# zhenpeiyang/RelativePose

Hardware: AMD Instinct MI355X
Metric: scan-pairs/sec end-to-end (completion+feat+spectral-match), 160x640 RGB-D (higher is better)
Workload: dtype f32 (fp32 products emulated on the bf16 matrix pipe: every operand cut into 3 bf16 pieces = its full 24 significand bits, the 6 partial products >= 2^-16 |ab| issued as v_mfma_f32_32x32x16_bf16, the 3 smallest dropped: a product error <= 2^-23 |ab| worst case, rms 2^-27.4 -- an fp32 multiply's own r

## Files before the change

include/relpose.h:

```cpp
#ifndef RELPOSE_H
#define RELPOSE_H

#include <stddef.h>
#include <stdint.h>

#ifdef __cplusplus
extern "C" {
#endif

#define RELPOSE_EINVAL (-1)
#define RELPOSE_ENOMEM (-2)
#define RELPOSE_EROUNDS (-3)

enum {
    RELPOSE_OK = 0,
    RELPOSE_FEW_KEYPOINTS = 1,
    RELPOSE_DIST_FILTER = 2,
    RELPOSE_ANGLE_FILTER = 3,
    RELPOSE_ZERO_WEIGHT = 4,
    RELPOSE_EDGE_OVERFLOW = 5,
    RELPOSE_NOT_CONVERGED = 6
};

enum { RELPOSE_SUNCG = 0, RELPOSE_MATTERPORT = 1, RELPOSE_SCANNET = 2 };
// ... 718 lines not shown
} RelposeSCNetConfig;
RelposeSCNet* relpose_scnet_create_ex(const RelposeSCNetConfig* cfg);

int relpose_scnet_set_param(RelposeSCNet* net, const char* key, const float* data_host, size_t numel);
int relpose_scnet_finalize(RelposeSCNet* net);
int64_t relpose_scnet_num_params(const RelposeSCNet* net);

enum { RELPOSE_PREC_F32 = 0, RELPOSE_PREC_BF16X3 = 1, RELPOSE_PREC_F16X3 = 2, RELPOSE_PREC_F16 = 3, RELPOSE_PREC_BF16X9 = 4, RELPOSE_PREC_BF16X6 = 5 };
int relpose_scnet_set_precision(RelposeSCNet* net, int32_t mode);

size_t relpose_scnet_workspace_bytes(const RelposeSCNet* net, int32_t n_images, int32_t H, int32_t W);

int relpose_scnet_forward(RelposeSCNet* net, const float* x, float* out, int32_t n_images, int32_t H, int32_t W,
                          void* workspace, size_t workspace_bytes, void* stream);

enum { RELPOSE_FWD_ZERO_WARP = 1, RELPOSE_FWD_POSE_OUTPUTS = 2, RELPOSE_FWD_NEW_WORKSPACE = 4 };
typedef struct RelposeForwardArgs {
    uint32_t struct_size;
    int32_t flags;
    const float* x;
    float* out;
    int32_t n_images, H, W, reserved0;
    void* workspace;
    size_t workspace_bytes;
    void* stream;
    void* tail_stream;
    uint64_t self_tag;
    uint64_t workspace_generation;
    void* reserved1;
} RelposeForwardArgs;
int relpose_scnet_forward_ex(RelposeSCNet* net, const RelposeForwardArgs* args);

int relpose_scnet_plan_macs(RelposeSCNet* net, int32_t n_images, int32_t flags, int32_t self_cached, double* macs_host);

int relpose_scnet_layer_kernel(RelposeSCNet* net, const char* layer, int32_t n_images);

int relpose_scnet_zero_tiles(RelposeSCNet* net, void* workspace, void* stream, int64_t* counts_host);

int relpose_scnet_conv1_zero(RelposeSCNet* net, void* workspace, void* stream, int64_t* counts_host, uint32_t* occ_host);

int relpose_scnet_conv4_rows(RelposeSCNet* net, void* workspace, void* stream, int64_t* counts_host);

int64_t relpose_scnet_read_tap(RelposeSCNet* net, const char* layer, float* out, void* workspace, void* stream);

int relpose_scnet_profile(RelposeSCNet* net, const float* x, float* out, int32_t n_images, int32_t H, int32_t W,
                          void* workspace, size_t workspace_bytes, int32_t iters,
// ... 7 lines not shown
```

relativepose_amd/_lib.py:

```python
import ctypes as C
import os

HERE = os.path.dirname(os.path.abspath(__file__))
LIB_PATH = os.environ.get("RELPOSE_LIB_PATH") or os.path.join(HERE, "librelpose_hip.so")

c_void_p, c_int, c_int64, c_size_t, c_double, c_char_p = C.c_void_p, C.c_int32, C.c_int64, C.c_size_t, C.c_double, C.c_char_p


class Params(C.Structure):
    _fields_ = [("distThre", c_double), ("distSepThre", c_double), ("angleThre", c_double),
                ("sigmaAngle1", c_double), ("sigmaAngle2", c_double), ("sigmaDist", c_double),
                ("sigmaFeat", c_double), ("mu", c_double), ("topK", c_int), ("method", c_int)]


class Keypoints(C.Structure):
    _fields_ = [("B", c_int), ("ns_max", c_int), ("nt_max", c_int),
                ("ns", c_void_p), ("nt", c_void_p),
                ("pc_s", c_void_p), ("normal_s", c_void_p), ("feat_s", c_void_p), ("weight_s", c_void_p),
                ("pc_t", c_void_p), ("normal_t", c_void_p), ("feat_t", c_void_p), ("weight_t", c_void_p)]


class MatchDebug(C.Structure):
    _fields_ = [("wij", c_void_p), ("corres_j", c_void_p), ("corres_w", c_void_p),
                ("counts", c_void_p), ("trace", c_void_p), ("eig_iters", c_void_p)]


class ForwardArgs(C.Structure):
    _fields_ = [("struct_size", C.c_uint32), ("flags", c_int), ("x", c_void_p), ("out", c_void_p),
                ("n_images", c_int), ("H", c_int), ("W", c_int), ("reserved0", c_int),
                ("workspace", c_void_p), ("workspace_bytes", c_size_t), ("stream", c_void_p), ("tail_stream", c_void_p),
                ("self_tag", C.c_uint64), ("workspace_generation", C.c_uint64), ("reserved1", c_void_p)]


class SCNetConfig(C.Structure):
    _fields_ = [("struct_size", C.c_uint32), ("snumclass", c_int), ("use_tanh", c_int), ("batchnorm", c_int), ("skip_layer", c_int),
                ("output_mask", c_int)]


class MatchArgs(C.Structure):
    _fields_ = [("struct_size", C.c_uint32), ("fit_cluster", c_int), ("params_host", C.POINTER(Params)), ("kp_host", C.POINTER(Keypoints)),
                ("workspace", c_void_p), ("workspace_bytes", c_size_t), ("max_edges", c_int64), ("pose", c_void_p), ("status", c_void_p),
                ("debug_host", C.POINTER(MatchDebug)), ("stream", c_void_p), ("affinity_kernel", c_int), ("reserved0", c_int)]


class SiftArgs(C.Structure):
    _fields_ = [("struct_size", C.c_uint32), ("n_views", c_int), ("images", c_void_p), ("img_h", c_int), ("img_w", c_int), ("channels", c_int),
# ... 275 lines not shown
    "relpose_pose_sync_workspace": (c_size_t, [c_int, c_int, c_int]),
    "relpose_pose_sync": (c_int, [C.POINTER(PoseSyncArgs)]),
    "relpose_scnet_create": (c_void_p, [c_int, c_int]),
    "relpose_scnet_create_ex": (c_void_p, [C.POINTER(SCNetConfig)]),
    "relpose_scnet_destroy": (None, [c_void_p]),
    "relpose_scnet_set_param": (c_int, [c_void_p, c_char_p, c_void_p, c_size_t]),
    "relpose_scnet_finalize": (c_int, [c_void_p]),
    "relpose_scnet_set_precision": (c_int, [c_void_p, c_int]),
    "relpose_scnet_num_params": (c_int64, [c_void_p]),
    "relpose_scnet_workspace_bytes": (c_size_t, [c_void_p, c_int, c_int, c_int]),
    "relpose_scnet_forward": (c_int, [c_void_p, c_void_p, c_void_p, c_int, c_int, c_int, c_void_p, c_size_t, c_void_p]),
    "relpose_scnet_forward_ex": (c_int, [c_void_p, C.POINTER(ForwardArgs)]),
    "relpose_scnet_plan_macs": (c_int, [c_void_p, c_int, c_int, c_int, C.POINTER(c_double)]),
    "relpose_scnet_layer_kernel": (c_int, [c_void_p, c_char_p, c_int]),
    "relpose_scnet_zero_tiles": (c_int, [c_void_p, c_void_p, c_void_p, C.POINTER(c_int64)]),
    "relpose_scnet_conv1_zero": (c_int, [c_void_p, c_void_p, c_void_p, C.POINTER(c_int64), c_void_p]),
    "relpose_scnet_conv4_rows": (c_int, [c_void_p, c_void_p, c_void_p, C.POINTER(c_int64)]),
    "relpose_scnet_read_tap": (c_int64, [c_void_p, c_char_p, c_void_p, c_void_p, c_void_p]),
    "relpose_scnet_profile": (c_int, [c_void_p, c_void_p, c_void_p, c_int, c_int, c_int, c_void_p, c_size_t, c_int,
                                      C.POINTER(c_double), C.POINTER(c_double), C.POINTER(c_int64), c_void_p]),
}

_lib = None


def lib():
    global _lib
    if _lib is None:
        if not os.path.exists(LIB_PATH):
            _build_locked()
# ... 71 lines not shown
```

relativepose_amd/csrc/geometry.hip:

```cpp
#include "common.h"
#include "rp_math.h"
#include "skybox.h"
#include <limits.h>

namespace {

struct Box { int y0, y1, x0, x1; };
__host__ __device__ inline Box observed_box(int method, int h) {
    Box b;
    if (method == RELPOSE_MASK_SECOND) { b.y0 = 0; b.y1 = h; b.x0 = h; b.x1 = 2 * h; }
    else {
        int dw = (int)(44 * (h / 160.0)), dh = (int)(33 * (h / 160.0));
        b.y0 = h / 2 - dh; b.y1 = h / 2 + dh; b.x0 = h + h / 2 - dw; b.x1 = h + h / 2 + dw;
    }
    return b;
}

__global__ void apply_mask_kernel(float* x, float* mask, int n, int c, int h, Box bx) {
    const size_t hw = (size_t)h * 4 * h;
    const size_t total = (size_t)n * hw;
    for (size_t idx = (size_t)blockIdx.x * blockDim.x + threadIdx.x; idx < total; idx += (size_t)gridDim.x * blockDim.x) {
        const size_t img = idx / hw, p = idx - img * hw;
        const int y = (int)(p / (4 * h)), xx = (int)(p - (size_t)y * 4 * h);
        const float m = (y >= bx.y0 && y < bx.y1 && xx >= bx.x0 && xx < bx.x1) ? 1.0f : 0.0f;
// ... 176 lines not shown

__global__ void sample_primitives_kernel(const float* __restrict__ f, int cf, int feat_off, const float* __restrict__ obs_norm,
                                         const float* __restrict__ obs_depth, const double* __restrict__ pts,
                                         const int* __restrict__ npts, int npts_max, double* __restrict__ pc,
                                         double* __restrict__ normal, float* __restrict__ feat, int n, int h, Box bx, int dataset,
                                         int compose) {
    const int img = blockIdx.y;
    const int k = blockIdx.x * blockDim.x + threadIdx.x;
    if (k >= npts[img]) return;
    const size_t hw = (size_t)h * 4 * h;
    const int W = 4 * h;
    const float* fi = f + (size_t)img * cf * hw;
    const float* on = obs_norm + (size_t)img * 3 * hw;
    const float* od = obs_depth + (size_t)img * hw;
    const double px = pts[((size_t)img * npts_max + k) * 2 + 0], py = pts[((size_t)img * npts_max + k) * 2 + 1];
    const int tx = (int)floor(px), ty = (int)floor(py);
    const double fx1 = px - tx, fx0 = tx + 1 - px, fy1 = py - ty, fy0 = ty + 1 - py;
    float n00[3], n01[3], n10[3], n11[3], d00, d01, d10, d11;
    composed_pixel(fi, cf, on, od, hw, h, bx, compose, ty, tx, n00, d00);
    composed_pixel(fi, cf, on, od, hw, h, bx, compose, ty, tx + 1, n01, d01);
    composed_pixel(fi, cf, on, od, hw, h, bx, compose, ty + 1, tx, n10, d10);
    composed_pixel(fi, cf, on, od, hw, h, bx, compose, ty + 1, tx + 1, n11, d11);
    const double val = (((double)d00 * fy0 * fx0 + (double)d01 * fx1 * fy0) + (double)d10 * fy1 * fx0) + (double)d11 * fx1 * fy1;
    double nn[3];
#pragma unroll
    for (int a = 0; a < 3; ++a)
        nn[a] = (((double)n00[a] * fy0 * fx0 + (double)n01[a] * fx1 * fy0) + (double)n10[a] * fy1 * fx0) + (double)n11[a] * fx1 * fy1;
    const double nl = rp_norm3(nn[0], nn[1], nn[2]);
    double* no = normal + ((size_t)img * npts_max + k) * 3;
    no[0] = nn[0] / nl; no[1] = nn[1] / nl; no[2] = nn[2] / nl;
    const int slot = (int)floor(px / h);
    const double ystp = (0.5 - py / h) * 2, xstp = ((px - slot * h) / h - 0.5) * 2;
    double ox, oy, oz;
    rp_face_rot(rp_face_index(dataset, slot), xstp * val, ystp * val, -val, ox, oy, oz);
    double* po = pc + ((size_t)img * npts_max + k) * 3;
    po[0] = ox; po[1] = oy; po[2] = oz;
    const float ptx = (float)(px / W), pty = (float)(py / h);
    const float x = ptx * (float)(W - 1), y = pty * (float)(h - 1);
    const float x0 = floorf(x), y0 = floorf(y);
    const int xi = (int)x0, yi = (int)y0;
    const float wx0 = x0 + 1.0f - x, wy0 = y0 + 1.0f - y, wx1 = x - x0, wy1 = y - y0;
    const float* ff = fi + (size_t)feat_off * hw;
    float* fo = feat + ((size_t)img * npts_max + k) * 32;
    for (int c = 0; c < 32; ++c) {
        const float* fc = ff + (size_t)c * hw;
        const float v00 = fc[(size_t)yi * W + xi], v10 = fc[(size_t)(yi + 1) * W + xi];
        const float v01 = fc[(size_t)yi * W + xi + 1], v11 = fc[(size_t)(yi + 1) * W + xi + 1];
        fo[c] = ((v00 * wx0 * wy0 + v10 * wx0 * wy1) + v01 * wx1 * wy0) + v11 * wx1 * wy1;
    }
}

__global__ void get_pixel_kernel(const double* __restrict__ depth, const double* __restrict__ normal, const double* __restrict__ pts,
                                 int k_total, int h, int dataset, double* __restrict__ pc, double* __restrict__ nn_out) {
    const int k = blockIdx.x * blockDim.x + threadIdx.x;
    if (k >= k_total) return;
// ... 321 lines not shown
```

relativepose_amd/csrc/scnet.hip:

```cpp
#include "common.h"
#include "matcher_internal.h"
#include "conv1_zero_geom.h"
#include <map>
#include <string>
#include <vector>
#include <algorithm>
#include <math.h>
#include <stdio.h>
#include <string.h>
#include <type_traits>
#include <stdlib.h>
#include <stddef.h>

namespace {

typedef float floatx16 __attribute__((ext_vector_type(16)));
typedef __bf16 bf16x8 __attribute__((ext_vector_type(8)));
typedef __bf16 bf16x4 __attribute__((ext_vector_type(4)));
typedef _Float16 f16x8 __attribute__((ext_vector_type(8)));
typedef _Float16 f16x4 __attribute__((ext_vector_type(4)));
template <int SPLIT> struct SplitT { typedef bf16x8 v8; typedef bf16x4 v4; };
template <> struct SplitT<2> { typedef f16x8 v8; typedef f16x4 v4; };
template <> struct SplitT<3> { typedef f16x8 v8; typedef f16x4 v4; };
typedef float rp_f4v __attribute__((ext_vector_type(4)));
// ... 2373 lines not shown
        if (ox < W) {
            int x0, x1; float lx0, lx1;
            lin_coef(ox, sww, RS, x0, x1, lx0, lx1);
            const float* a = srow + (x0 - g.sx) * C;
            const float* b = srow + (x1 - g.sx) * C;
            const float* cc = a + RO_MAXW * C;
            const float* dd = b + RO_MAXW * C;
            float* o = y + (size_t)g.img * C * H * W + (size_t)g.oy * W + ox;
            for (int c = 0; c < C; ++c)
                o[(size_t)c * H * W] = g.ly0 * (lx0 * a[c] + lx1 * b[c]) + g.ly1 * (lx0 * cc[c] + lx1 * dd[c]);
        }
        __builtin_amdgcn_wave_barrier();
    }
}

struct Phase {
    int ntaps; signed char offy[16], offx[16];
    int py, px, Hp, Wp;
    size_t w_off;
    size_t ws_off = 0;
    size_t wh_off = 0;
    float wh_scale = 1.f;
    size_t w3_off = 0;
    int K;
};

struct Layer {
    std::string name;
    int kind;
    int cin, cout, k, stride, pad;
// ... 9 lines not shown
struct RelposeSCNet {
    int S, use_tanh, cf;
    int bn = 1, skip = 1, omask = 31;
    bool variant() const { return !(bn && skip && omask == 31); }
    std::map<std::string, std::vector<float>> params;
    std::map<std::string, std::vector<int64_t>> shapes;
    bool finalized = false;
    int prec = 0;
    int64_t nparams = 0;
    float* d_w = nullptr;
    float* d_gb = nullptr;
    float2* d_ident = nullptr;
    size_t w1_off = 0;
    size_t wh_off = 0, bh_off = 0;
    std::map<std::pair<void*, int64_t>, void*> plans;
    struct SelfState { uint64_t tag = 0, gen = 0; int n = 0, H = 0, W = 0; int snap_heads = 0; bool c4_rows = false; };
    std::map<void*, SelfState> self_state;
    std::map<std::string, Layer> layers;
    std::map<std::string, Buf> bufs;
    size_t per_image_floats = 0, ss_float2_per_group = 0;
    size_t gb_floats = 0;
    int last_n = 0;
    const int* last_zt_counts = nullptr;
    const int* last_c4_hdr = nullptr;
    int last_c4_nimg[6] = {0, 0, 0, 0, 0, 0};
    int64_t last_zt_units[2] = {0, 0};
    bool w1_finite = false;
    struct A1zState { uint64_t gen = 0; int n = 0, H = 0, W = 0; };
    std::map<void*, A1zState> a1z_state;
    int64_t last_c1_units = 0;
    bool last_c1_codes = false, last_occ = false;
    bool profiling = false;
    std::vector<hipEvent_t> ev;
    std::vector<int> ev_kind;
};

namespace {
// ... 903 lines not shown
                          size_t workspace_bytes, void* stream) {
    const RelposeForwardArgs a = rp_fwd_args(x, out, n, H, W, workspace, workspace_bytes, stream, stream, 0, 0);
    return relpose_scnet_forward_ex(net, &a);
}

int relpose_scnet_forward_ex(RelposeSCNet* net, const RelposeForwardArgs* args) {
    if (!net || !args || args->struct_size < offsetof(RelposeForwardArgs, self_tag)) return RELPOSE_EINVAL;
    const float* x = args->x; float* out = args->out;
    const int32_t n = args->n_images, H = args->H, W = args->W, flags = args->flags;
    void* workspace = args->workspace; const size_t workspace_bytes = args->workspace_bytes;
    const bool variant = net->variant();
    void* stream = args->stream; void* tail_stream = (args->tail_stream && !variant) ? args->tail_stream : args->stream;
    const uint64_t self_tag = (!variant && args->struct_size >= offsetof(RelposeForwardArgs, self_tag) + sizeof(uint64_t)) ? args->self_tag : 0;
    const uint64_t ws_gen = args->struct_size >= offsetof(RelposeForwardArgs, workspace_generation) + sizeof(uint64_t) ? args->workspace_generation : 0;
    if (!net->finalized || !x || !out || !workspace || n <= 0 || (n & 1) || H <= 0 || W <= 0 || n >= (1 << 24)) return RELPOSE_EINVAL;
    if (flags & ~(RELPOSE_FWD_ZERO_WARP | RELPOSE_FWD_POSE_OUTPUTS | RELPOSE_FWD_NEW_WORKSPACE)) return RELPOSE_EINVAL;
    if (args->struct_size >= offsetof(RelposeForwardArgs, reserved1) + sizeof(void*) && args->reserved1) return RELPOSE_EINVAL;
    const int G = n / 2;
    const bool zero_warp = (flags & RELPOSE_FWD_ZERO_WARP) && n > 2 && !variant;
    const bool pose_only = (flags & RELPOSE_FWD_POSE_OUTPUTS) != 0 && !variant;
    Plan* plan = nullptr;
    RelposeSCNet::SelfState commit;
    const bool zt_on = g_rp_tune[RELPOSE_TUNE_ZERO_TILES] != 1;
    const bool c4_on = zt_on && g_rp_tune[RELPOSE_TUNE_CONV4_ROWS] != 1;
    commit.c4_rows = c4_on;
    commit.tag = self_tag; commit.n = n; commit.H = H; commit.W = W; commit.gen = ws_gen;
    if (flags & RELPOSE_FWD_NEW_WORKSPACE) net->self_state.erase(workspace);
    RelposeSCNet::SelfState prev = net->self_state[workspace];
    net->self_state[workspace] = RelposeSCNet::SelfState();
    bool self_cached = self_tag != 0 && prev.tag == self_tag && prev.n == n && prev.H == H && prev.W == W && (prev.snap_heads & 6) == 6 && !zero_warp &&
                       prev.gen == ws_gen && prev.c4_rows == c4_on;
    int snap_mode = 0, snap_heads = 7;
    const int ds_key = ((g_rp_tune[RELPOSE_TUNE_DECONV_STRIP] == 1 ? 1 : 0) << 28) | ((zt_on ? 0 : 1) << 29) | ((c4_on ? 0 : 1) << 30);
    auto key_of = [&]() {
        return (int64_t)((int)n | (zero_warp ? 1 << 24 : 0) | (pose_only ? 1 << 25 : 0) | (self_cached ? 1 << 26 : 0) | (snap_mode == 1 ? 1 << 27 : 0) | ds_key) |
// ... 22 lines not shown
        B.zt = zt_on ? (int*)(ws + o.zt) + zt_occ_ints(n) : nullptr;
        B.c4r = c4_on ? (int*)(ws + o.c4r) : nullptr;
        build_plan(net, n, B);
        if (B.rc) {
            delete p;
            if (self_cached) { self_cached = false; continue; }
            return B.rc;
        }
        RP_HIP(hipMalloc((void**)&p->d_descs, MAX_DESCS * sizeof(ConvDesc)));
        RP_HIP(hipMemcpy(p->d_descs, p->descs.data(), p->descs.size() * sizeof(ConvDesc), hipMemcpyHostToDevice));
        net->plans[std::make_pair(workspace, key_of())] = p;
        plan = p;
    }
    if (!plan) return RELPOSE_EINVAL;
    commit.snap_heads = plan->self_cached ? prev.snap_heads : (self_tag != 0 ? (pose_only ? 6 : 7) : 0);
    net->last_n = n;
    const bool two = tail_stream != stream;
    hipStream_t s = (two && plan->head_count > 0) ? (hipStream_t)tail_stream : (hipStream_t)stream;
    const WsOffsets o = ws_offsets(net, n);
    char* ws = (char*)workspace;
    float* act = (float*)(ws + o.act);
    float2* ssp = (float2*)(ws + o.ss);
    double* partial = (double*)(ws + o.partial);
    auto mark = [&](int kind) {
        if (!net->profiling) return;
        hipEvent_t e; (void)hipEventCreate(&e); (void)hipEventRecord(e, s);
        net->ev.push_back(e); net->ev_kind.push_back(kind);
    };
    if (net->omask != 31) {
        for (const char* bn_ : {"D3", "D2", "OUT"}) {
            const Buf& B = net->bufs[bn_];
// ... 170 lines not shown
            mark(2);
            hipLaunchKernelGGL(bn_finalize_fused_kernel, dim3((B.C + 31) / 32, G), dim3(1024), 0, s, plan->d_descs + op.first, op.count, op.skip_blk,
                               B.C, 2 * B.H * B.H, net->d_gb + B.gb_off, net->d_gb + B.gb_off + B.C, ssp + B.ss_off * G);
            mark(-2);
        } else if (op.type == OP_SS_FILL) {
            const Buf& B = net->bufs[op.buf];
            mark(2);
            hipLaunchKernelGGL(ss_fill_kernel, dim3((B.C * G + 255) / 256), dim3(256), 0, s, B.C, G, net->d_gb + B.gb_off, net->d_gb + B.gb_off + B.C,
                               ssp + B.ss_off * G);
            mark(-2);
        } else if (op.type == OP_BCAST) {
            const Buf& B = net->bufs[op.buf];
            mark(2);
            hipLaunchKernelGGL(bcast_warped_kernel, dim3(2048), dim3(256), 0, s, act + B.off * n, n, B.H * B.H, B.C, B.C / 6, ssp + B.ss_off * G, G);
            mark(-2);
        } else if (op.type == OP_HEADS) {
            HeadsDesc hd;
            hd.d2 = act + net->bufs["D2"].off * n; hd.a1 = act + net->bufs["A1"].off * n;
            hd.ss_d2 = ssp + net->bufs["D2"].ss_off * G; hd.ss_a1 = ssp + net->bufs["A1"].ss_off * G;
            hd.w = net->d_w + net->wh_off; hd.bias = net->d_w + net->bh_off; hd.out = act + net->bufs["OUT"].off * n;
            hd.n = n; hd.S = net->S; hd.cf = net->cf; hd.use_tanh = net->use_tanh;
            hd.snap_mode = plan->snap_mode; hd.snap = (float*)(ws + o.snap) + plan->heads_snap_off; hd.snap_heads = plan->snap_heads;
            mark(1);
            const dim3 hg((unsigned)((size_t)n * RS * RS / 256));
#define RP_HEADS_LAUNCH(S_, POSE_)                                                                                         \
            { if (lanepix) hipLaunchKernelGGL((heads_lanepix_kernel<S_, POSE_>), hg, dim3(256), 0, s, hd);               \
              else hipLaunchKernelGGL((heads_kernel<S_, POSE_>), hg, dim3(256), 0, s, hd); }
            const bool lanepix = g_rp_tune[RELPOSE_TUNE_HEADS_KERNEL] == 1;
            if (plan->pose_only) {
                if (net->S == 15) RP_HEADS_LAUNCH(15, true) else RP_HEADS_LAUNCH(21, true)
            } else if (net->S == 15) RP_HEADS_LAUNCH(15, false) else RP_HEADS_LAUNCH(21, false)
#undef RP_HEADS_LAUNCH
            mark(-1);
        } else if (op.type == OP_REDUCE) {
            mark(4);
            if (op.cfg == 1) {
                const ConvDesc& d0 = plan->descs[op.first];
// ... 22 lines not shown
            int nch = (2048 + G - 1) / G;
            if (nch > (rows + 63) / 64) nch = (rows + 63) / 64;
            if (nch > 64) nch = 64;
            if (nch < 1) nch = 1;
            const int chunk_rows = (rows + nch - 1) / nch;
            nch = (rows + chunk_rows - 1) / chunk_rows;
            const int q4 = B.C / 4, nrl = 256 / q4;
            mark(2);
            hipLaunchKernelGGL(bn_partial_kernel, dim3(nch, G), dim3(256), (size_t)nrl * q4 * 8 * sizeof(double), s, act + B.off * n, rows,
                               B.C, chunk_rows, partial);
            hipLaunchKernelGGL(bn_finalize_kernel, dim3((B.C + 255) / 256, G), dim3(256), 0, s, partial, nch, B.C, rows,
                               net->d_gb + B.gb_off, net->d_gb + B.gb_off + B.C, ssp + B.ss_off * G);
            mark(-2);
        }
    }
    mark(3);
    hipLaunchKernelGGL(resize_out_kernel, dim3(4096), dim3(256), net->cf <= RO_MAXC ? (size_t)4 * 2 * RO_MAXW * net->cf * sizeof(float) : 0, s,
                       act + net->bufs["OUT"].off * n, out, n, net->cf, H, W);
    mark(-3);
    RP_CHECK_LAUNCH();
    {
        net->self_state[workspace] = commit;
        if (net->last_c1_codes) {
            RelposeSCNet::A1zState z; z.gen = ws_gen; z.n = n; z.H = H; z.W = W;
            net->a1z_state[workspace] = z;
        }
    }
    return 0;
}

int relpose_scnet_plan_macs(RelposeSCNet* net, int32_t n, int32_t flags, int32_t self_cached, double* macs_out) {
    if (!net || !net->finalized || !macs_out || n <= 0 || (n & 1)) return RELPOSE_EINVAL;
    if (net->variant()) { flags = 0; self_cached = 0; }
    const bool zero_warp = (flags & RELPOSE_FWD_ZERO_WARP) && n > 2 && !self_cached;
    const bool pose_only = (flags & RELPOSE_FWD_POSE_OUTPUTS) != 0;
    Plan dry;
    Builder B; B.net = net; B.n = n; B.G = n / 2; B.act = nullptr; B.ss = nullptr; B.splitk = nullptr; B.statp = nullptr; B.plan = &dry;
    B.zero_warp = zero_warp; B.pose_only = pose_only; B.self_cached = self_cached != 0;
    B.snapbuf = (float*)(uintptr_t)4096;
    B.snap_mode = self_cached ? 2 : 1; dry.snap_mode = B.snap_mode;
    const int snap_heads = self_cached == 2 ? 6 : 7;
    B.snap_heads = snap_heads; dry.snap_heads = snap_heads;
    build_plan(net, n, B);
    if (B.rc) return B.rc;
    double macs = 0;
    for (const Op& op : dry.ops) {
        if (op.type == OP_CONV || op.type == OP_CONV_S2 || op.type == OP_CONV_STRIP || op.type == OP_DECONV_TILE) {
            for (int i = op.first; i < op.first + op.count; ++i) {
                const ConvDesc& d = dry.descs[i];
                double rowsK;
                if (op.type == OP_CONV_STRIP && d.ksplit > 1 && (d.shared_slices || d.skip_slices)) {
                    rowsK = 0;
                    for (int ks = 0; ks < d.ksplit; ++ks) {
                        if ((d.skip_slices >> ks) & 1) continue;
                        const double rows = ((d.shared_slices >> ks) & 1) ? 2.0 * d.Hp * d.Wp : (double)d.M;
                        rowsK += rows * d.K / d.ksplit;
                    }
                } else if (op.type == OP_DECONV_TILE && d.nsrc == 2 && plan_snap_mode(dry, i) == 2) {
                    rowsK = (double)d.M * d.ntaps * d.src[0].C;
                } else rowsK = (double)d.M * d.K;
                macs += rowsK * d.Cout;
            }
        } else if (op.type == OP_CONV1) {
            const double blk = 224.0 * 224 * 32 * (36 + 36 + 18);
            const double self_imgs = self_cached ? 0 : n, warp_imgs = zero_warp ? 2 : n;
            macs += blk * (self_imgs + warp_imgs);
        } else if (op.type == OP_HEADS) {
            const double px = (double)n * 224 * 224;
            const int hc[5] = {3, 3, 1, net->S, 32};
            for (int m = 0; m < 5; ++m) {
                if (pose_only && (m == 0 || m == 3)) continue;
                const int cin = (m < 3 && self_cached && ((snap_heads >> m) & 1)) ? 32 : 64;
                macs += px * cin * hc[m];
            }
        }
    }
    *macs_out = macs;
    return 0;
}

int relpose_scnet_layer_kernel(RelposeSCNet* net, const char* layer, int32_t n) {
    if (!net || !net->finalized || !layer || n <= 0 || (n & 1)) return RELPOSE_EINVAL;
    Plan dry;
    Builder B; B.net = net; B.n = n; B.G = n / 2; B.act = nullptr; B.ss = nullptr; B.splitk = nullptr; B.statp = nullptr; B.plan = &dry;
    B.probe_layer = layer;
    build_plan(net, n, B);
    if (B.rc) return B.rc;
    if (B.probe_desc < 0) return RELPOSE_EINVAL;
    for (const Op& op : dry.ops)
        if ((op.type == OP_CONV || op.type == OP_CONV_S2 || op.type == OP_CONV_STRIP || op.type == OP_DECONV_TILE) && B.probe_desc >= op.first &&
            B.probe_desc < op.first + op.count)
            return (op.type == OP_CONV_STRIP && op.cfg == 1) ? (dry.descs[B.probe_desc].ksplit == 1 ? 2 : 1) : 0;
    return RELPOSE_EINVAL;
}
// ... 103 lines not shown
```

relativepose_amd/model.py:

```python
import ctypes as C

import numpy as np
import torch

from . import _lib
from .weights import HEADS, head_channels, parse_output_type, state_dict_spec

PRECISION_CODES = {"f32": 0, "bf16x3": 1, "f16x3": 2, "f16": 3, "bf16x9": 4, "bf16x6": 5}

BUFFER_SHAPES = {"X0": (224, 16), "A1": (224, 192), "A2": (112, 384), "A3": (56, 768), "A4": (28, 256), "A5": (14, 512),
                 "A6": (7, 512), "A7": (3, 512), "A8": (3, 512), "A9": (1, 1024), "D9": (3, 512), "D8": (3, 512),
                 "D7": (7, 512), "D6": (14, 512), "D5": (28, 256), "D4": (56, 128), "D3": (112, 320), "D2": (224, 224)}


_REGISTRY = {}


class SCNet(torch.nn.Module):

    def __init__(self, args):
        super().__init__()
        self.snumclass = int(args.snumclass)
        self.useTanh = int(getattr(args, "useTanh", 1))
        self.batchnorm = int(bool(getattr(args, "batchnorm", 1)))
# ... 102 lines not shown
        self._wss[key] = ent
        ws, self._ws_gen = ent
        ws.record_stream(torch.cuda.current_stream())
        for s in also_streams:
            ws.record_stream(s)
        self._ws, self._ws_n = ws, n
        return ws

    _tag_counter = 0

    @classmethod
    def new_self_tag(cls):
        cls._tag_counter += 1
        return cls._tag_counter

    FLAG_ZERO_WARP, FLAG_POSE_OUTPUTS, FLAG_NEW_WORKSPACE = 1, 2, 4

    def forward(self, x, out=None, tail_stream=None, ws_key=None, zero_warp=False, outputs="all", self_tag=0):
        flags = (self.FLAG_ZERO_WARP if zero_warp else 0) | {"all": 0, "pose": self.FLAG_POSE_OUTPUTS}[outputs]
        return self.forward_flags(x, out, flags, self_tag, tail_stream, ws_key)

    def forward_flags(self, x, out=None, flags=0, self_tag=0, tail_stream=None, ws_key=None):
        import torch
        _lib.require_gpu()
        if not self._loaded:
            raise RuntimeError("load_state_dict first")
        assert x.is_cuda and x.dtype == torch.float32 and x.dim() == 4 and x.shape[1] == 16
        x = x.contiguous()
        n, _, H, W = x.shape
        if isinstance(tail_stream, int):
            tail_stream = None if tail_stream == 0 else torch.cuda.ExternalStream(tail_stream)
        ws = self._workspace(n, H, W, x.device, ws_key, tuple(s_ for s_ in (tail_stream,) if s_ is not None))
        if tail_stream is not None:
            x.record_stream(tail_stream)
        user_out = None
        if self.is_variant:
            tail_stream, user_out = None, out
            out = torch.empty(n, self.full_channels, H, W, dtype=torch.float32, device=x.device)
        elif out is None:
            out = torch.empty(n, self.out_channels, H, W, dtype=torch.float32, device=x.device)
            if tail_stream is not None:
                out.record_stream(tail_stream)
        else:
            assert out.is_cuda and out.dtype == torch.float32 and out.is_contiguous() and tuple(out.shape) == (n, self.out_channels, H, W)
        a = _lib.ForwardArgs()
        a.struct_size = C.sizeof(_lib.ForwardArgs)
        a.flags = int(flags) & 7
        a.x, a.out = x.data_ptr(), out.data_ptr()
        a.n_images, a.H, a.W = n, H, W
        a.workspace, a.workspace_bytes = ws.data_ptr(), ws.numel()
        a.stream = torch.cuda.current_stream().cuda_stream
        a.tail_stream = a.stream if tail_stream is None else tail_stream.cuda_stream
        a.self_tag = int(self_tag)
        a.workspace_generation = self._ws_gen
        _lib.check(_lib.lib().relpose_scnet_forward_ex(self._h, C.byref(a)), "relpose_scnet_forward_ex")
        if self.is_variant:
            sel = out if self.out_channels == self.full_channels else out[:, self._sel]
            if user_out is None:
                return sel.contiguous()
            user_out.copy_(sel)
            return user_out
        return out
# ... 59 lines not shown
```

relativepose_amd/pipeline.py:

```python
import numpy as np

from . import _lib, rpmodule, util


class RelativePosePipeline:
    _chain_nets = False
    _net_stream = None
    _net_streams = None

    def __init__(self, net, dataset="suncg", mask_method="second", sigmas=None, alter_steps=3, completion=1, max_edges=0, compose=0, outputs="all",
                 self_stream_cache=True, tail_overlap=True, net_priority=None, loop_fit_cluster=1, keypoints="given", level_outputs="last"):
        self.net = net
        if keypoints not in ("given", "reference"):
            raise ValueError("keypoints must be 'given' or 'reference'")
        self.keypoints = keypoints
        self.self_stream_cache = self_stream_cache
        self.outputs = outputs
        if level_outputs not in ("last", "every"):
            raise ValueError("level_outputs must be 'last' or 'every'")
        self.level_outputs = level_outputs
        self.dataset = dataset
        self.mask_method = mask_method
        self.alter_steps = alter_steps
        self.completion = completion
        self.max_edges = max_edges
        self.compose = compose
        if sigmas is None:
            o = rpmodule.opts()
            sigmas = [[o.sigmaAngle1, o.sigmaAngle2, o.sigmaDist, o.sigmaFeat]] * alter_steps
        self.sigmas = np.asarray(sigmas, dtype=np.float64).reshape(-1, 4)
        self.feat_off = 7 + net.snumclass
        self._slot_streams = []
        self.tail_overlap = bool(tail_overlap)
        self.net_priority = net_priority
        self.loop_fit_cluster = int(loop_fit_cluster)
# ... 237 lines not shown
                        results[k] = on_result(k, pose, status)
                    else:
                        if provider is not None:
                            cur.wait_stream(st["stream"])
                            cur.wait_stream(self._net_stream)
                        results[k] = (pose, status)
        for st in states:
            if "stream" in st:
                cur.wait_stream(st["stream"])
        for ss in self._slot_streams[:depth]:
            cur.wait_stream(ss)
        cur.wait_stream(self._net_stream)
        self._chain_nets = False
        return results

    def _outputs_at(self, step, keep=None):
        if self.outputs == "all" and self.level_outputs == "last" and keep is None and step < self.alter_steps - 1 and not self.net.is_variant:
            return "pose"
        return self.outputs

    def _net_input(self, st):
        import torch
        B, h = st["B"], st["h"]
        view = util.build_view_dev(st["rgb"], st["norm"], st["depth"], self.mask_method)
        x = st.get("x")
        if x is None:
            x = st["x"] = torch.empty(2 * B, 16, h, 4 * h, dtype=torch.float32, device=view.device)
        x[:, :8].copy_(view)
        st["self_tag"] = self.net.new_self_tag() if self.self_stream_cache else 0
        f = st.get("f")
        if f is None or f.shape[1] != self.net.out_channels:
            st["f"] = torch.empty(2 * B, self.net.out_channels, h, 4 * h, dtype=torch.float32, device=view.device)
# ... 2 lines not shown
    def _run_gen(self, st):
        import torch
        B, h, N = st["B"], st["h"], st["N"]
        x = self._net_input(st)
        R_hat, status = st["eye"], None
        for step in range(self.alter_steps):
            inv = R_hat if step == 0 else util.pose_inverse_dev(R_hat)
            poses = torch.stack((inv, R_hat), 1).reshape(2 * B, 4, 4).contiguous()
            util.warp_pairs_dev(x, poses, self.dataset)
            if self._chain_nets:
                ms, ns = torch.cuda.current_stream(), self._net_stream
                ns.wait_stream(ms)
                if self.tail_overlap:
                    f = st["f"]
                    with torch.cuda.stream(ns):
                        self.net.forward(x, out=f, tail_stream=ms, ws_key=ms.cuda_stream, zero_warp=(step == 0), outputs=self._outputs_at(step),
                                         self_tag=st["self_tag"])
                else:
                    with torch.cuda.stream(ns):
                        f = self.net.forward(x, out=st["f"], zero_warp=(step == 0), outputs=self._outputs_at(step), self_tag=st["self_tag"])
                        done = torch.cuda.Event()
                        done.record()
                    ms.wait_event(done)
                yield
            else:
                f = self.net.forward(x, out=st["f"], zero_warp=(step == 0), outputs=self._outputs_at(step), self_tag=st["self_tag"])
            kpts, knpts, w_s, w_t, ns, nt = self._level_keypoints(st, f, step)
            pc, nn, ft = util.sample_primitives_dev(f, self.feat_off, st["norm"], st["depth"], kpts, knpts,
                                                    self.mask_method, self.dataset, self.compose)
            pc, nn, ft = pc.view(B, 2, N, 3), nn.view(B, 2, N, 3), ft.view(B, 2, N, 32)
            para = rpmodule.opts(*self.sigmas[min(step, len(self.sigmas) - 1)])
            res = rpmodule.match_pairs(pc[:, 0].contiguous(), nn[:, 0].contiguous(), ft[:, 0].contiguous(), w_s,
                                       pc[:, 1].contiguous(), nn[:, 1].contiguous(), ft[:, 1].contiguous(), w_t,
                                       ns, nt, para, max_edges=self.max_edges, fit_cluster=self.loop_fit_cluster if self._chain_nets else 0)
            R_hat, status = res.pose, res.status
        return R_hat, status, None

    def run(self, st, R_forced=None, keep=None, primitives=None):
        import torch
        B, h, N = st["B"], st["h"], st["N"]
        x = self._net_input(st)
        R_hat = st["eye"]
        trace = []
        status = None
        for step in range(self.alter_steps):
            if R_forced is not None:
                R_hat = R_forced[step]
            inv = R_hat if (step == 0 and R_forced is None) else util.pose_inverse_dev(R_hat)
            poses = torch.stack((inv, R_hat), 1).reshape(2 * B, 4, 4).contiguous()
            util.warp_pairs_dev(x, poses, self.dataset)
            f = self.net.forward(x, out=st["f"] if keep is None else None, zero_warp=(step == 0 and R_forced is None),
                                 outputs=self._outputs_at(step, keep), self_tag=st["self_tag"])
            kpts, knpts, w_s, w_t, ns, nt = self._level_keypoints(st, f, step)
            pc, nn, ft = util.sample_primitives_dev(f, self.feat_off, st["norm"], st["depth"], kpts, knpts,
                                                    self.mask_method, self.dataset, self.compose)
            pc, nn, ft = pc.view(B, 2, N, 3), nn.view(B, 2, N, 3), ft.view(B, 2, N, 32)
            para = rpmodule.opts(*self.sigmas[min(step, len(self.sigmas) - 1)])
            res = rpmodule.match_pairs(pc[:, 0].contiguous(), nn[:, 0].contiguous(), ft[:, 0].contiguous(), w_s,
                                       pc[:, 1].contiguous(), nn[:, 1].contiguous(), ft[:, 1].contiguous(), w_t,
                                       ns, nt, para, max_edges=self.max_edges)
            R_hat, status = res.pose, res.status
            trace.append(R_hat)
            if primitives is not None:
                primitives.update(pc=pc, nn=nn, ft=ft, step=step, w_s=w_s, w_t=w_t, ns=ns, nt=nt)
            if keep is not None:
                keep.append({"x": x.clone(), "f": f, "pc": pc, "nn": nn, "ft": ft, "pts": kpts.view(B, 2, N, 2), "w_s": w_s, "w_t": w_t, "ns": ns, "nt": nt})
        return R_hat, status, trace
# ... 1 lines not shown
```

Baseline: 1039.

## Compute output heads only at sampled keypoint pixels for intermediate levels

Adds a sampled-outputs forward mode. For non-final alternation steps it runs the normal/depth and feature heads only at the 2x2 neighbourhoods of given keypoints, through a new per-keypoint kernel, and skips the dense heads and the full-resolution resize. This removes dense head GEMMs and the resize pass over every pixel on intermediate levels. In exchange, the dense output buffer stays stale outside the sampled pixels. Heads-snapshot bookkeeping is adjusted so the next dense call does not reuse snapshots that were never produced.

```diff
diff --git a/include/relpose.h b/include/relpose.h
--- a/include/relpose.h
+++ b/include/relpose.h
@@ -756,7 +756,7 @@
 int relpose_scnet_forward(RelposeSCNet* net, const float* x, float* out, int32_t n_images, int32_t H, int32_t W,
                           void* workspace, size_t workspace_bytes, void* stream);
 
-enum { RELPOSE_FWD_ZERO_WARP = 1, RELPOSE_FWD_POSE_OUTPUTS = 2, RELPOSE_FWD_NEW_WORKSPACE = 4 };
+enum { RELPOSE_FWD_ZERO_WARP = 1, RELPOSE_FWD_POSE_OUTPUTS = 2, RELPOSE_FWD_NEW_WORKSPACE = 4, RELPOSE_FWD_SAMPLED_OUTPUTS = 32 };
 typedef struct RelposeForwardArgs {
     uint32_t struct_size;
     int32_t flags;
@@ -770,8 +770,13 @@
     uint64_t self_tag;
     uint64_t workspace_generation;
     void* reserved1;
+    const double* sample_pts;
+    const int32_t* sample_npts;
+    int32_t sample_npts_max, reserved2;
 } RelposeForwardArgs;
 int relpose_scnet_forward_ex(RelposeSCNet* net, const RelposeForwardArgs* args);
+
+int relpose_scnet_last_tail(RelposeSCNet* net);
 
 int relpose_scnet_plan_macs(RelposeSCNet* net, int32_t n_images, int32_t flags, int32_t self_cached, double* macs_host);
 
diff --git a/relativepose_amd/_lib.py b/relativepose_amd/_lib.py
--- a/relativepose_amd/_lib.py
+++ b/relativepose_amd/_lib.py
@@ -29,7 +29,8 @@
     _fields_ = [("struct_size", C.c_uint32), ("flags", c_int), ("x", c_void_p), ("out", c_void_p),
                 ("n_images", c_int), ("H", c_int), ("W", c_int), ("reserved0", c_int),
                 ("workspace", c_void_p), ("workspace_bytes", c_size_t), ("stream", c_void_p), ("tail_stream", c_void_p),
-                ("self_tag", C.c_uint64), ("workspace_generation", C.c_uint64), ("reserved1", c_void_p)]
+                ("self_tag", C.c_uint64), ("workspace_generation", C.c_uint64), ("reserved1", c_void_p),
+                ("sample_pts", c_void_p), ("sample_npts", c_void_p), ("sample_npts_max", c_int), ("reserved2", c_int)]
 
 
 class SCNetConfig(C.Structure):
@@ -335,6 +336,7 @@
     "relpose_scnet_plan_macs": (c_int, [c_void_p, c_int, c_int, c_int, C.POINTER(c_double)]),
     "relpose_scnet_layer_kernel": (c_int, [c_void_p, c_char_p, c_int]),
     "relpose_scnet_zero_tiles": (c_int, [c_void_p, c_void_p, c_void_p, C.POINTER(c_int64)]),
+    "relpose_scnet_last_tail": (c_int, [c_void_p]),
     "relpose_scnet_conv1_zero": (c_int, [c_void_p, c_void_p, c_void_p, C.POINTER(c_int64), c_void_p]),
     "relpose_scnet_conv4_rows": (c_int, [c_void_p, c_void_p, c_void_p, C.POINTER(c_int64)]),
     "relpose_scnet_read_tap": (c_int64, [c_void_p, c_char_p, c_void_p, c_void_p, c_void_p]),
diff --git a/relativepose_amd/csrc/geometry.hip b/relativepose_amd/csrc/geometry.hip
--- a/relativepose_amd/csrc/geometry.hip
+++ b/relativepose_amd/csrc/geometry.hip
@@ -1,5 +1,6 @@
 #include "common.h"
 #include "rp_math.h"
+#include "sample_pixels.h"
 #include "skybox.h"
 #include <limits.h>
 
@@ -214,7 +215,8 @@
     const float* on = obs_norm + (size_t)img * 3 * hw;
     const float* od = obs_depth + (size_t)img * hw;
     const double px = pts[((size_t)img * npts_max + k) * 2 + 0], py = pts[((size_t)img * npts_max + k) * 2 + 1];
-    const int tx = (int)floor(px), ty = (int)floor(py);
+    const RpSamplePix sp = rp_sample_pixels(px, py, h);
+    const int tx = sp.tx, ty = sp.ty;
     const double fx1 = px - tx, fx0 = tx + 1 - px, fy1 = py - ty, fy0 = ty + 1 - py;
     float n00[3], n01[3], n10[3], n11[3], d00, d01, d10, d11;
     composed_pixel(fi, cf, on, od, hw, h, bx, compose, ty, tx, n00, d00);
@@ -235,10 +237,8 @@
     rp_face_rot(rp_face_index(dataset, slot), xstp * val, ystp * val, -val, ox, oy, oz);
     double* po = pc + ((size_t)img * npts_max + k) * 3;
     po[0] = ox; po[1] = oy; po[2] = oz;
-    const float ptx = (float)(px / W), pty = (float)(py / h);
-    const float x = ptx * (float)(W - 1), y = pty * (float)(h - 1);
-    const float x0 = floorf(x), y0 = floorf(y);
-    const int xi = (int)x0, yi = (int)y0;
+    const float x = sp.x, y = sp.y, x0 = sp.x0, y0 = sp.y0;
+    const int xi = sp.xi, yi = sp.yi;
     const float wx0 = x0 + 1.0f - x, wy0 = y0 + 1.0f - y, wx1 = x - x0, wy1 = y - y0;
     const float* ff = fi + (size_t)feat_off * hw;
     float* fo = feat + ((size_t)img * npts_max + k) * 32;
diff --git a/relativepose_amd/csrc/sample_pixels.h b/relativepose_amd/csrc/sample_pixels.h
--- /dev/null
+++ b/relativepose_amd/csrc/sample_pixels.h
@@ -0,0 +1,14 @@
+#pragma once
+#include "rp_math.h"
+
+struct RpSamplePix { int tx, ty, xi, yi; float x, y, x0, y0; };
+RP_HD RpSamplePix rp_sample_pixels(double px, double py, int h) {
+    const int W = 4 * h;
+    RpSamplePix s;
+    s.tx = (int)floor(px); s.ty = (int)floor(py);
+    const float ptx = (float)(px / W), pty = (float)(py / h);
+    s.x = ptx * (float)(W - 1); s.y = pty * (float)(h - 1);
+    s.x0 = floorf(s.x); s.y0 = floorf(s.y);
+    s.xi = (int)s.x0; s.yi = (int)s.y0;
+    return s;
+}
diff --git a/relativepose_amd/csrc/scnet.hip b/relativepose_amd/csrc/scnet.hip
--- a/relativepose_amd/csrc/scnet.hip
+++ b/relativepose_amd/csrc/scnet.hip
@@ -1,6 +1,7 @@
 #include "common.h"
 #include "matcher_internal.h"
 #include "conv1_zero_geom.h"
+#include "sample_pixels.h"
 #include <map>
 #include <string>
 #include <vector>
@@ -2411,6 +2412,104 @@
     }
 }
 
+struct SampledDesc {
+    const float* d2; const float* a1; const float2* ss_d2; const float2* ss_a1;
+    const float* w; const float* bias; float* out;
+    const double* pts; const int* npts;
+    int npts_max, cf, use_tanh, H, W;
+};
+
+__global__ __launch_bounds__(256) void heads_sampled_kernel(const SampledDesc sd) {
+    __shared__ float ndl[4][16][4];
+    __shared__ float fl[4][16][32];
+    const int lane = threadIdx.x & 63, wave = threadIdx.x >> 6;
+    const int img = blockIdx.y, k = blockIdx.x * 4 + wave;
+    if (k >= sd.npts_max || k >= sd.npts[img]) return;
+    const int H = sd.H, W = sd.W, cf = sd.cf, feat_off = cf - 32;
+    const double px = sd.pts[((size_t)img * sd.npts_max + k) * 2 + 0], py = sd.pts[((size_t)img * sd.npts_max + k) * 2 + 1];
+    const RpSamplePix sp = rp_sample_pixels(px, py, H);
+    const float shh = (float)RS / H, sww = (float)RS / W;
+    const int g = img >> 1;
+    const float2* ssd = sd.ss_d2 + (size_t)g * 224;
+    const float2* ssa = sd.ss_a1 + (size_t)g * 192;
+    auto item_src = [&](int item, int by, int bx, int& oy, int& ox, size_t& spix) {
+        oy = by + (item >> 3); ox = bx + ((item >> 2) & 1);
+        if (oy < 0 || oy >= H || ox < 0 || ox >= W) return false;
+        int y0, y1, x0, x1; float ly0, ly1, lx0, lx1;
+        lin_coef(oy, shh, RS, y0, y1, ly0, ly1);
+        lin_coef(ox, sww, RS, x0, x1, lx0, lx1);
+        spix = ((size_t)img * RS + ((item & 2) ? y1 : y0)) * RS + ((item & 1) ? x1 : x0);
+        return true;
+    };
+    if (lane < 16) {
+        int oy, ox; size_t spix;
+        if (item_src(lane, sp.ty, sp.tx, oy, ox, spix)) {
+            const float* pa = sd.a1 + spix * 192;
+            const float* pd = sd.d2 + spix * 224;
+            float an[3] = {0.f, 0.f, 0.f}, ad = 0.f;
+            for (int c = 0; c < 32; ++c) {
+                const float2 sc = ssa[64 + c];
+                const float v = lrelu(pa[64 + c] * sc.x + sc.y, LRELU);
+                for (int j = 0; j < 3; ++j) an[j] = __builtin_fmaf(v, sd.w[(128 + c) * 4 + j], an[j]);
+            }
+            for (int c = 0; c < 32; ++c) {
+                const float2 sc = ssa[128 + c];
+                const float v = lrelu(pa[128 + c] * sc.x + sc.y, LRELU);
+                ad = __builtin_fmaf(v, sd.w[(160 + c) * 4], ad);
+            }
+            for (int c = 0; c < 32; ++c) {
+                const float2 sc = ssd[32 + c];
+                const float v = lrelu(pd[32 + c] * sc.x + sc.y, LRELU);
+                for (int j = 0; j < 3; ++j) an[j] = __builtin_fmaf(v, sd.w[(32 + c) * 4 + j], an[j]);
+            }
+            for (int c = 0; c < 32; ++c) {
+                const float2 sc = ssd[64 + c];
+                const float v = lrelu(pd[64 + c] * sc.x + sc.y, LRELU);
+                ad = __builtin_fmaf(v, sd.w[(64 + c) * 4], ad);
+            }
+            for (int j = 0; j < 3; ++j) ndl[wave][lane][j] = an[j] + sd.bias[3 + j];
+            ndl[wave][lane][3] = ad + sd.bias[6];
+        }
+    } else if (lane < 48) {
+        const int item = (lane - 16) & 15, o0 = ((lane - 16) >> 4) * 16;
+        int oy, ox; size_t spix;
+        if (item_src(item, sp.yi, sp.xi, oy, ox, spix)) {
+            const float* pd = sd.d2 + spix * 224 + 160;
+            const float* wf = sd.w + 2304 + o0;
+            float af[16];
+#pragma unroll
+            for (int o = 0; o < 16; ++o) af[o] = 0.f;
+            for (int c = 0; c < 64; ++c) {
+                const float2 sc = ssd[160 + c];
+                const float v = lrelu(pd[c] * sc.x + sc.y, LRELU);
+#pragma unroll
+                for (int o = 0; o < 16; ++o) af[o] = __builtin_fmaf(v, wf[c * 32 + o], af[o]);
+            }
+#pragma unroll
+            for (int o = 0; o < 16; ++o) {
+                const float v = af[o] + sd.bias[feat_off + o0 + o];
+                fl[wave][item][o0 + o] = sd.use_tanh ? tanhf(v) : v;
+            }
+        }
+    }
+    rp_wave_lds_sync();
+    const size_t hw = (size_t)H * W;
+    float* const oi = sd.out + (size_t)img * cf * hw;
+    for (int e = lane; e < 16 + 128; e += 64) {
+        const bool nd = e < 16;
+        const int p = nd ? (e >> 2) : ((e - 16) >> 5), c = nd ? (e & 3) : ((e - 16) & 31);
+        const int oy = (nd ? sp.ty : sp.yi) + (p >> 1), ox = (nd ? sp.tx : sp.xi) + (p & 1);
+        if (oy < 0 || oy >= H || ox < 0 || ox >= W) continue;
+        int y0, y1, x0, x1; float ly0, ly1, lx0, lx1;
+        lin_coef(oy, shh, RS, y0, y1, ly0, ly1);
+        lin_coef(ox, sww, RS, x0, x1, lx0, lx1);
+        const float a = nd ? ndl[wave][p * 4 + 0][c] : fl[wave][p * 4 + 0][c], b = nd ? ndl[wave][p * 4 + 1][c] : fl[wave][p * 4 + 1][c];
+        const float cc = nd ? ndl[wave][p * 4 + 2][c] : fl[wave][p * 4 + 2][c], dd = nd ? ndl[wave][p * 4 + 3][c] : fl[wave][p * 4 + 3][c];
+        const float r = __fmaf_rn(ly0, __fmaf_rn(lx0, a, __fmul_rn(lx1, b)), __fmul_rn(ly1, __fmaf_rn(lx0, cc, __fmul_rn(lx1, dd))));
+        oi[(size_t)(nd ? 3 + c : feat_off + c) * hw + (size_t)oy * W + ox] = r;
+    }
+}
+
 struct Phase {
     int ntaps; signed char offy[16], offx[16];
     int py, px, Hp, Wp;
@@ -2450,13 +2549,14 @@
     size_t w1_off = 0;
     size_t wh_off = 0, bh_off = 0;
     std::map<std::pair<void*, int64_t>, void*> plans;
-    struct SelfState { uint64_t tag = 0, gen = 0; int n = 0, H = 0, W = 0; int snap_heads = 0; bool c4_rows = false; };
+    struct SelfState { uint64_t tag = 0, gen = 0; int n = 0, H = 0, W = 0; int snap_heads = 0; int heads_snap = 0; bool c4_rows = false; };
     std::map<void*, SelfState> self_state;
     std::map<std::string, Layer> layers;
     std::map<std::string, Buf> bufs;
     size_t per_image_floats = 0, ss_float2_per_group = 0;
     size_t gb_floats = 0;
     int last_n = 0;
+    int last_tail = -1;
     const int* last_zt_counts = nullptr;
     const int* last_c4_hdr = nullptr;
     int last_c4_nimg[6] = {0, 0, 0, 0, 0, 0};
@@ -3390,11 +3490,17 @@
     const uint64_t self_tag = (!variant && args->struct_size >= offsetof(RelposeForwardArgs, self_tag) + sizeof(uint64_t)) ? args->self_tag : 0;
     const uint64_t ws_gen = args->struct_size >= offsetof(RelposeForwardArgs, workspace_generation) + sizeof(uint64_t) ? args->workspace_generation : 0;
     if (!net->finalized || !x || !out || !workspace || n <= 0 || (n & 1) || H <= 0 || W <= 0 || n >= (1 << 24)) return RELPOSE_EINVAL;
-    if (flags & ~(RELPOSE_FWD_ZERO_WARP | RELPOSE_FWD_POSE_OUTPUTS | RELPOSE_FWD_NEW_WORKSPACE)) return RELPOSE_EINVAL;
+    if (flags & ~(RELPOSE_FWD_ZERO_WARP | RELPOSE_FWD_POSE_OUTPUTS | RELPOSE_FWD_NEW_WORKSPACE | RELPOSE_FWD_SAMPLED_OUTPUTS)) return RELPOSE_EINVAL;
+    const bool sampled = (flags & RELPOSE_FWD_SAMPLED_OUTPUTS) != 0 && !variant;
+    if (flags & RELPOSE_FWD_SAMPLED_OUTPUTS) {
+        if (args->struct_size < offsetof(RelposeForwardArgs, sample_npts_max) + sizeof(int32_t)) return RELPOSE_EINVAL;
+        if (!args->sample_pts || !args->sample_npts || args->sample_npts_max <= 0 || W != 4 * H) return RELPOSE_EINVAL;
+        if (!variant && net->S != 15 && net->S != 21) return RELPOSE_EINVAL;
+    }
     if (args->struct_size >= offsetof(RelposeForwardArgs, reserved1) + sizeof(void*) && args->reserved1) return RELPOSE_EINVAL;
     const int G = n / 2;
     const bool zero_warp = (flags & RELPOSE_FWD_ZERO_WARP) && n > 2 && !variant;
-    const bool pose_only = (flags & RELPOSE_FWD_POSE_OUTPUTS) != 0 && !variant;
+    const bool pose_only = ((flags & RELPOSE_FWD_POSE_OUTPUTS) != 0 && !variant) || sampled;
     Plan* plan = nullptr;
     RelposeSCNet::SelfState commit;
     const bool zt_on = g_rp_tune[RELPOSE_TUNE_ZERO_TILES] != 1;
@@ -3447,7 +3553,9 @@
     }
     if (!plan) return RELPOSE_EINVAL;
     commit.snap_heads = plan->self_cached ? prev.snap_heads : (self_tag != 0 ? (pose_only ? 6 : 7) : 0);
+    commit.heads_snap = plan->self_cached ? prev.heads_snap : (sampled ? 0 : commit.snap_heads);
     net->last_n = n;
+    net->last_tail = sampled ? 1 : 0;
     const bool two = tail_stream != stream;
     hipStream_t s = (two && plan->head_count > 0) ? (hipStream_t)tail_stream : (hipStream_t)stream;
     const WsOffsets o = ws_offsets(net, n);
@@ -3648,6 +3756,16 @@
             mark(2);
             hipLaunchKernelGGL(bcast_warped_kernel, dim3(2048), dim3(256), 0, s, act + B.off * n, n, B.H * B.H, B.C, B.C / 6, ssp + B.ss_off * G, G);
             mark(-2);
+        } else if (op.type == OP_HEADS && sampled) {
+            SampledDesc sd;
+            sd.d2 = act + net->bufs["D2"].off * n; sd.a1 = act + net->bufs["A1"].off * n;
+            sd.ss_d2 = ssp + net->bufs["D2"].ss_off * G; sd.ss_a1 = ssp + net->bufs["A1"].ss_off * G;
+            sd.w = net->d_w + net->wh_off; sd.bias = net->d_w + net->bh_off; sd.out = out;
+            sd.pts = args->sample_pts; sd.npts = args->sample_npts; sd.npts_max = args->sample_npts_max;
+            sd.cf = net->cf; sd.use_tanh = net->use_tanh; sd.H = H; sd.W = W;
+            mark(1);
+            hipLaunchKernelGGL(heads_sampled_kernel, dim3((unsigned)((args->sample_npts_max + 3) / 4), (unsigned)n), dim3(256), 0, s, sd);
+            mark(-1);
         } else if (op.type == OP_HEADS) {
             HeadsDesc hd;
             hd.d2 = act + net->bufs["D2"].off * n; hd.a1 = act + net->bufs["A1"].off * n;
@@ -3655,6 +3773,10 @@
             hd.w = net->d_w + net->wh_off; hd.bias = net->d_w + net->bh_off; hd.out = act + net->bufs["OUT"].off * n;
             hd.n = n; hd.S = net->S; hd.cf = net->cf; hd.use_tanh = net->use_tanh;
             hd.snap_mode = plan->snap_mode; hd.snap = (float*)(ws + o.snap) + plan->heads_snap_off; hd.snap_heads = plan->snap_heads;
+            if (hd.snap_mode == 2) {
+                hd.snap_heads &= prev.heads_snap | (plan->pose_only ? 1 : 0);
+                if ((hd.snap_heads & 6) != 6) { hd.snap_mode = 0; hd.snap_heads = 7; }
+            }
             mark(1);
             const dim3 hg((unsigned)((size_t)n * RS * RS / 256));
 #define RP_HEADS_LAUNCH(S_, POSE_)                                                                                         \
@@ -3707,10 +3829,12 @@
             mark(-2);
         }
     }
-    mark(3);
-    hipLaunchKernelGGL(resize_out_kernel, dim3(4096), dim3(256), net->cf <= RO_MAXC ? (size_t)4 * 2 * RO_MAXW * net->cf * sizeof(float) : 0, s,
-                       act + net->bufs["OUT"].off * n, out, n, net->cf, H, W);
-    mark(-3);
+    if (!sampled) {
+        mark(3);
+        hipLaunchKernelGGL(resize_out_kernel, dim3(4096), dim3(256), net->cf <= RO_MAXC ? (size_t)4 * 2 * RO_MAXW * net->cf * sizeof(float) : 0, s,
+                           act + net->bufs["OUT"].off * n, out, n, net->cf, H, W);
+        mark(-3);
+    }
     RP_CHECK_LAUNCH();
     {
         net->self_state[workspace] = commit;
@@ -3726,13 +3850,15 @@
     if (!net || !net->finalized || !macs_out || n <= 0 || (n & 1)) return RELPOSE_EINVAL;
     if (net->variant()) { flags = 0; self_cached = 0; }
     const bool zero_warp = (flags & RELPOSE_FWD_ZERO_WARP) && n > 2 && !self_cached;
-    const bool pose_only = (flags & RELPOSE_FWD_POSE_OUTPUTS) != 0;
+    const bool sampled = (flags & RELPOSE_FWD_SAMPLED_OUTPUTS) != 0;
+    const bool pose_only = (flags & RELPOSE_FWD_POSE_OUTPUTS) != 0 || sampled;
     Plan dry;
     Builder B; B.net = net; B.n = n; B.G = n / 2; B.act = nullptr; B.ss = nullptr; B.splitk = nullptr; B.statp = nullptr; B.plan = &dry;
     B.zero_warp = zero_warp; B.pose_only = pose_only; B.self_cached = self_cached != 0;
     B.snapbuf = (float*)(uintptr_t)4096;
     B.snap_mode = self_cached ? 2 : 1; dry.snap_mode = B.snap_mode;
-    const int snap_heads = self_cached == 2 ? 6 : 7;
+    const int snap_heads = (self_cached == 2 || self_cached == 3) ? 6 : 7;
+    const int heads_snap = self_cached == 3 ? 0 : snap_heads;
     B.snap_heads = snap_heads; dry.snap_heads = snap_heads;
     build_plan(net, n, B);
     if (B.rc) return B.rc;
@@ -3758,12 +3884,12 @@
             const double blk = 224.0 * 224 * 32 * (36 + 36 + 18);
             const double self_imgs = self_cached ? 0 : n, warp_imgs = zero_warp ? 2 : n;
             macs += blk * (self_imgs + warp_imgs);
-        } else if (op.type == OP_HEADS) {
+        } else if (op.type == OP_HEADS && !sampled) {
             const double px = (double)n * 224 * 224;
             const int hc[5] = {3, 3, 1, net->S, 32};
             for (int m = 0; m < 5; ++m) {
                 if (pose_only && (m == 0 || m == 3)) continue;
-                const int cin = (m < 3 && self_cached && ((snap_heads >> m) & 1)) ? 32 : 64;
+                const int cin = (m < 3 && self_cached && ((heads_snap >> m) & 1)) ? 32 : 64;
                 macs += px * cin * hc[m];
             }
         }
@@ -3771,6 +3897,8 @@
     *macs_out = macs;
     return 0;
 }
+
+int relpose_scnet_last_tail(RelposeSCNet* net) { return net ? net->last_tail : RELPOSE_EINVAL; }
 
 int relpose_scnet_layer_kernel(RelposeSCNet* net, const char* layer, int32_t n) {
     if (!net || !net->finalized || !layer || n <= 0 || (n & 1)) return RELPOSE_EINVAL;
diff --git a/relativepose_amd/model.py b/relativepose_amd/model.py
--- a/relativepose_amd/model.py
+++ b/relativepose_amd/model.py
@@ -140,13 +140,19 @@
         cls._tag_counter += 1
         return cls._tag_counter
 
-    FLAG_ZERO_WARP, FLAG_POSE_OUTPUTS, FLAG_NEW_WORKSPACE = 1, 2, 4
-
-    def forward(self, x, out=None, tail_stream=None, ws_key=None, zero_warp=False, outputs="all", self_tag=0):
-        flags = (self.FLAG_ZERO_WARP if zero_warp else 0) | {"all": 0, "pose": self.FLAG_POSE_OUTPUTS}[outputs]
-        return self.forward_flags(x, out, flags, self_tag, tail_stream, ws_key)
-
-    def forward_flags(self, x, out=None, flags=0, self_tag=0, tail_stream=None, ws_key=None):
+    FLAG_ZERO_WARP, FLAG_POSE_OUTPUTS, FLAG_NEW_WORKSPACE, FLAG_SAMPLED_OUTPUTS = 1, 2, 4, 32
+
+    def forward(self, x, out=None, tail_stream=None, ws_key=None, zero_warp=False, outputs="all", self_tag=0, sample_pts=None, sample_npts=None):
+        flags = (self.FLAG_ZERO_WARP if zero_warp else 0) | {"all": 0, "pose": self.FLAG_POSE_OUTPUTS, "samples": self.FLAG_SAMPLED_OUTPUTS}[outputs]
+        if outputs == "samples" and (sample_pts is None or sample_npts is None):
+            raise ValueError("outputs='samples' needs sample_pts and sample_npts")
+        return self.forward_flags(x, out, flags, self_tag, tail_stream, ws_key, sample_pts if outputs == "samples" else None, sample_npts)
+
+    def last_tail(self):
+        r = int(_lib.lib().relpose_scnet_last_tail(self._h))
+        return {0: "dense", 1: "sampled"}.get(r)
+
+    def forward_flags(self, x, out=None, flags=0, self_tag=0, tail_stream=None, ws_key=None, sample_pts=None, sample_npts=None):
         import torch
         _lib.require_gpu()
         if not self._loaded:
@@ -171,7 +177,17 @@
             assert out.is_cuda and out.dtype == torch.float32 and out.is_contiguous() and tuple(out.shape) == (n, self.out_channels, H, W)
         a = _lib.ForwardArgs()
         a.struct_size = C.sizeof(_lib.ForwardArgs)
-        a.flags = int(flags) & 7
+        a.flags = int(flags) & (7 | self.FLAG_SAMPLED_OUTPUTS)
+        if a.flags & self.FLAG_SAMPLED_OUTPUTS:
+            if sample_pts is None or sample_npts is None:
+                raise ValueError("RELPOSE_FWD_SAMPLED_OUTPUTS needs sample_pts and sample_npts")
+            assert sample_pts.is_cuda and sample_pts.dtype == torch.float64 and sample_pts.is_contiguous() and sample_pts.dim() == 3
+            assert tuple(sample_pts.shape) == (n, sample_pts.shape[1], 2) and sample_pts.shape[1] > 0
+            assert sample_npts.is_cuda and sample_npts.dtype == torch.int32 and sample_npts.is_contiguous() and tuple(sample_npts.shape) == (n,)
+            a.sample_pts, a.sample_npts, a.sample_npts_max = sample_pts.data_ptr(), sample_npts.data_ptr(), int(sample_pts.shape[1])
+            if tail_stream is not None:
+                sample_pts.record_stream(tail_stream)
+                sample_npts.record_stream(tail_stream)
         a.x, a.out = x.data_ptr(), out.data_ptr()
         a.n_images, a.H, a.W = n, H, W
         a.workspace, a.workspace_bytes = ws.data_ptr(), ws.numel()
diff --git a/relativepose_amd/pipeline.py b/relativepose_amd/pipeline.py
--- a/relativepose_amd/pipeline.py
+++ b/relativepose_amd/pipeline.py
@@ -9,7 +9,8 @@
     _net_streams = None
 
     def __init__(self, net, dataset="suncg", mask_method="second", sigmas=None, alter_steps=3, completion=1, max_edges=0, compose=0, outputs="all",
-                 self_stream_cache=True, tail_overlap=True, net_priority=None, loop_fit_cluster=1, keypoints="given", level_outputs="last"):
+                 self_stream_cache=True, tail_overlap=True, net_priority=None, loop_fit_cluster=1, keypoints="given", level_outputs="last",
+                 sampled_levels=True):
         self.net = net
         if keypoints not in ("given", "reference"):
             raise ValueError("keypoints must be 'given' or 'reference'")
@@ -19,6 +20,7 @@
         if level_outputs not in ("last", "every"):
             raise ValueError("level_outputs must be 'last' or 'every'")
         self.level_outputs = level_outputs
+        self.sampled_levels = bool(sampled_levels)
         self.dataset = dataset
         self.mask_method = mask_method
         self.alter_steps = alter_steps
@@ -286,8 +288,10 @@
         self._chain_nets = False
         return results
 
-    def _outputs_at(self, step, keep=None):
+    def _outputs_at(self, step, keep=None, st=None):
         if self.outputs == "all" and self.level_outputs == "last" and keep is None and step < self.alter_steps - 1 and not self.net.is_variant:
+            if self.sampled_levels and self.keypoints == "given" and st is not None and st["N"] > 0 and st["h"] * 4 == st["x"].shape[3]:
+                return "samples"
             return "pose"
         return self.outputs
 
@@ -320,17 +324,19 @@
                 if self.tail_overlap:
                     f = st["f"]
                     with torch.cuda.stream(ns):
-                        self.net.forward(x, out=f, tail_stream=ms, ws_key=ms.cuda_stream, zero_warp=(step == 0), outputs=self._outputs_at(step),
-                                         self_tag=st["self_tag"])
+                        self.net.forward(x, out=f, tail_stream=ms, ws_key=ms.cuda_stream, zero_warp=(step == 0), outputs=self._outputs_at(step, None, st),
+                                         self_tag=st["self_tag"], sample_pts=st.get("pts"), sample_npts=st.get("npts"))
                 else:
                     with torch.cuda.stream(ns):
-                        f = self.net.forward(x, out=st["f"], zero_warp=(step == 0), outputs=self._outputs_at(step), self_tag=st["self_tag"])
+                        f = self.net.forward(x, out=st["f"], zero_warp=(step == 0), outputs=self._outputs_at(step, None, st), self_tag=st["self_tag"],
+                                             sample_pts=st.get("pts"), sample_npts=st.get("npts"))
                         done = torch.cuda.Event()
                         done.record()
                     ms.wait_event(done)
                 yield
             else:
-                f = self.net.forward(x, out=st["f"], zero_warp=(step == 0), outputs=self._outputs_at(step), self_tag=st["self_tag"])
+                f = self.net.forward(x, out=st["f"], zero_warp=(step == 0), outputs=self._outputs_at(step, None, st), self_tag=st["self_tag"],
+                                             sample_pts=st.get("pts"), sample_npts=st.get("npts"))
             kpts, knpts, w_s, w_t, ns, nt = self._level_keypoints(st, f, step)
             pc, nn, ft = util.sample_primitives_dev(f, self.feat_off, st["norm"], st["depth"], kpts, knpts,
                                                     self.mask_method, self.dataset, self.compose)
@@ -356,7 +362,8 @@
             poses = torch.stack((inv, R_hat), 1).reshape(2 * B, 4, 4).contiguous()
             util.warp_pairs_dev(x, poses, self.dataset)
             f = self.net.forward(x, out=st["f"] if keep is None else None, zero_warp=(step == 0 and R_forced is None),
-                                 outputs=self._outputs_at(step, keep), self_tag=st["self_tag"])
+                                 outputs=self._outputs_at(step, keep, st), self_tag=st["self_tag"], sample_pts=st.get("pts"),
+                                 sample_npts=st.get("npts"))
             kpts, knpts, w_s, w_t, ns, nt = self._level_keypoints(st, f, step)
             pc, nn, ft = util.sample_primitives_dev(f, self.feat_off, st["norm"], st["depth"], kpts, knpts,
                                                     self.mask_method, self.dataset, self.compose)
```

Result: faster. 1097 (median of 6 runs) (+5.6%).
